# sudo-flow/zvec

Measured on AMD Instinct MI355X. Metric: QPS @ recall@10>=0.99, 10Mx768 fp32, batch=1024, higher is better.
Workload: dtype f32

## Files before the change

zvec_amd/csrc/api_entry_ctx_flat.inc.h:

```cpp

int zvec_hip_abi_version(void) { return ZVEC_HIP_ABI_VERSION; }

int zvec_hip_device_count(int *count) {
  if (!count) return ZVEC_HIP_ERR_INVALID_ARGUMENT;
  int n = 0;
  if (hipGetDeviceCount(&n) != hipSuccess) { *count = 0; return ZVEC_HIP_ERR_RUNTIME; }
  *count = n;
  return 0;
}

const char *zvec_hip_error_string(int code) {
  switch (code) {
    case ZVEC_HIP_OK: return "Success";
    case ZVEC_HIP_ERR_RUNTIME: return "Runtime error";
    case ZVEC_HIP_ERR_UNSUPPORTED: return "Unsupported";
    case ZVEC_HIP_ERR_OUT_OF_RANGE: return "Out of range";
    case ZVEC_HIP_ERR_NO_MEMORY: return "Not enough space";
    case ZVEC_HIP_ERR_NO_READY: return "No ready";
    case ZVEC_HIP_ERR_NO_EXIST: return "No exist";
    case ZVEC_HIP_ERR_MISMATCH: return "Mismatch";
    case ZVEC_HIP_ERR_INVALID_ARGUMENT: return "Invalid argument";
    case ZVEC_HIP_ERR_NO_INDEX_LOADED: return "No index loaded";
    case ZVEC_HIP_ERR_NO_TRAINED: return "No trained";
  }
  return "Unknown error";
}

int zvec_hip_set_option(const char *name, int value) {
  if (!name) return ZVEC_HIP_ERR_INVALID_ARGUMENT;
  if (strcmp(name, "wait") == 0) {
    if (value < 0 || value > 2) return ZVEC_HIP_ERR_INVALID_ARGUMENT;
    ropts().wait = value;
    return 0;
  }
  if (strcmp(name, "zerocopy") == 0) {
    if (value < 0 || value > 3) return ZVEC_HIP_ERR_INVALID_ARGUMENT;
    ropts().zerocopy = value;
    return 0;
  }
  if (strcmp(name, "assign256") == 0) { ropts().assign256 = value != 0; return 0; }
  if (strcmp(name, "scan256") == 0) {
    if (value < 0 || value > 2) return ZVEC_HIP_ERR_INVALID_ARGUMENT;
    ropts().scan256 = value;
    return 0;
  }
  if (strcmp(name, "sparse_group_rows") == 0) {
    if (value < 0 || value > 64) return ZVEC_HIP_ERR_INVALID_ARGUMENT;
    ropts().sparse_group_rows = value;
    return 0;
  }
  if (strcmp(name, "sparse_inverted_build") == 0) {
    if (value < 0 || value > 1) return ZVEC_HIP_ERR_INVALID_ARGUMENT;
    ropts().sparse_inverted_build = value;
    return 0;
  }
  return ZVEC_HIP_ERR_UNSUPPORTED;
}
int zvec_hip_get_option(const char *name, int *value) {
  if (!name || !value) return ZVEC_HIP_ERR_INVALID_ARGUMENT;
  if (strcmp(name, "wait") == 0) { *value = ropts().wait; return 0; }
  if (strcmp(name, "zerocopy") == 0) { *value = ropts().zerocopy; return 0; }
  if (strcmp(name, "assign256") == 0) { *value = ropts().assign256; return 0; }
  if (strcmp(name, "scan256") == 0) { *value = ropts().scan256; return 0; }
  if (strcmp(name, "sparse_group_rows") == 0) { *value = ropts().sparse_group_rows; return 0; }
  if (strcmp(name, "sparse_inverted_build") == 0) { *value = ropts().sparse_inverted_build; return 0; }
  return ZVEC_HIP_ERR_UNSUPPORTED;
}

int zvec_hip_host_alloc(uint64_t bytes, void **out) {
  if (!out || bytes == 0) return ZVEC_HIP_ERR_INVALID_ARGUMENT;
  void *p = nullptr;
  if (hipHostMalloc(&p, bytes, hipHostMallocPortable) != hipSuccess) { (void)hipGetLastError(); return ZVEC_HIP_ERR_NO_MEMORY; }
  *out = p;
  return 0;
}
int zvec_hip_host_free(void *p) {
  if (p) (void)hipHostFree(p);
  return 0;
}

int zvec_hip_ctx_create(int device, zvec_hip_ctx_t *out) {
  if (!out) return ZVEC_HIP_ERR_INVALID_ARGUMENT;
  return ctx_new(device, out);
}
int zvec_hip_ctx_destroy(zvec_hip_ctx_t ctx) { ctx_free(ctx); return 0; }
int zvec_hip_ctx_synchronize(zvec_hip_ctx_t ctx) {
  if (!ctx) return ZVEC_HIP_ERR_INVALID_ARGUMENT;
  ZCHK(hipSetDevice(ctx->device));
  ZCHK(hipStreamSynchronize(ctx->cur));
  return 0;
}
int zvec_hip_ctx_set_stream(zvec_hip_ctx_t ctx, void *stream) {
  if (!ctx) return ZVEC_HIP_ERR_INVALID_ARGUMENT;
  ctx->cur = stream ? reinterpret_cast<hipStream_t>(stream) : ctx->own;
  return 0;
}

int zvec_hip_gate_create(int device, zvec_hip_gate_t *out) {
  if (!out) return ZVEC_HIP_ERR_INVALID_ARGUMENT;
  ZCHK(hipSetDevice(device));
  zvec_hip_gate_s *g = new (std::nothrow) zvec_hip_gate_s();
  if (!g) return ZVEC_HIP_ERR_NO_MEMORY;
  g->device = device;
  if (hipEventCreateWithFlags(&g->ev, hipEventDisableTiming) != hipSuccess) { delete g; return ZVEC_HIP_ERR_RUNTIME; }
  *out = g;
  return 0;
}
int zvec_hip_gate_destroy(zvec_hip_gate_t g) {
  if (!g) return 0;
  (void)hipSetDevice(g->device);
  if (g->ev) (void)hipEventDestroy(g->ev);
  delete g;
  return 0;
}
int zvec_hip_ctx_set_gate(zvec_hip_ctx_t ctx, zvec_hip_gate_t gate) {
  if (!ctx || (gate && gate->device != ctx->device)) return ZVEC_HIP_ERR_INVALID_ARGUMENT;
  std::lock_guard<std::mutex> g(ctx->mu);
  ctx->gate = gate;
  return 0;
}

int zvec_hip_flat_create(uint32_t dim, int dtype, int metric, int device, zvec_hip_flat_t *out) {
  if (!out || dim == 0) return ZVEC_HIP_ERR_INVALID_ARGUMENT;
  if (dtype < ZVEC_HIP_DT_FP32 || dtype > ZVEC_HIP_DT_BINARY64) return ZVEC_HIP_ERR_UNSUPPORTED;
  if (metric < 0 || metric > ZVEC_HIP_METRIC_HAMMING) return ZVEC_HIP_ERR_UNSUPPORTED;
  if (dtype_is_binary(dtype) != (metric == ZVEC_HIP_METRIC_HAMMING)) return ZVEC_HIP_ERR_MISMATCH;
  if (dtype_is_binary(dtype) && (dim % (dtype == ZVEC_HIP_DT_BINARY64 ? 64u : 32u) != 0 || dim > (1u << 20))) return ZVEC_HIP_ERR_INVALID_ARGUMENT;
  if (metric == ZVEC_HIP_METRIC_COSINE && dim < (dtype == ZVEC_HIP_DT_FP16 ? 3u : 2u)) return ZVEC_HIP_ERR_INVALID_ARGUMENT;
  zvec_hip_ctx_s *c = nullptr;
  ZRET(ctx_new(device, &c));
  zvec_hip_flat_s *h = new (std::nothrow) zvec_hip_flat_s();
  if (!h) { ctx_free(c); return ZVEC_HIP_ERR_NO_MEMORY; }
  h->device = device; h->dtype = dtype; h->defctx = c;
  h->st.configure(dim, metric, dtype);
  *out = h;
  return 0;
}

int zvec_hip_flat_destroy(zvec_hip_flat_t h) {
  if (!h) return 0;
  (void)hipSetDevice(h->device);
  (void)hipDeviceSynchronize();
  delete h;
  return 0;
}

int zvec_hip_flat_reserve(zvec_hip_flat_t h, uint64_t capacity) {
  if (!h) return ZVEC_HIP_ERR_INVALID_ARGUMENT;
// ... 556 lines not shown
```

zvec_amd/csrc/api_flat_scan.inc.h:

```cpp

namespace {

struct KernelInfo {
  bool init = false;
  int cus = 0;
};
KernelInfo g_info[16];
std::mutex g_info_mu;

struct Knobs {
  int max_ng = 4;
  bool no_wide = false;
  bool force_wide = false;
  bool no_seed = false;
  bool no_gather = false;
  int ivf_tpc = 0;
  bool m16_small = true;
  int ivf_head_pct = 50;
  int ivf_occ_cap = 0;
  bool no_wide_dump = false;
  int ivf_direct_q = 8;
  int seed_rows256 = 16384;
  Knobs() {
#ifdef ZVEC_HIP_TUNING
    if (const char *e = getenv("ZVEC_HIP_MAX_NG")) max_ng = std::max(1, std::min(4, atoi(e)));
    no_wide = getenv("ZVEC_HIP_NO_WIDE") != nullptr;
    force_wide = getenv("ZVEC_HIP_FORCE_WIDE") != nullptr;
    no_seed = getenv("ZVEC_HIP_NO_SEED") != nullptr;
    no_gather = getenv("ZVEC_HIP_NO_GATHER") != nullptr;
    if (const char *e = getenv("ZVEC_HIP_IVF_TPC")) ivf_tpc = std::max(1, atoi(e));
    m16_small = getenv("ZVEC_HIP_NO_M16_SMALL") == nullptr;
    no_wide_dump = getenv("ZVEC_HIP_NO_WIDE_DUMP") != nullptr;
    if (const char *e = getenv("ZVEC_HIP_IVF_OCC_CAP")) ivf_occ_cap = std::max(0, atoi(e));
    if (const char *e = getenv("ZVEC_HIP_IVF_HEAD_PCT")) ivf_head_pct = std::max(0, std::min(75, atoi(e)));
    if (const char *e = getenv("ZVEC_HIP_IVF_DIRECT_Q")) ivf_direct_q = std::max(0, atoi(e));
    if (const char *e = getenv("ZVEC_HIP_SEED_ROWS256")) seed_rows256 = std::max(128, atoi(e) / 128 * 128);
#endif
  }
};
const Knobs &knobs() {
  static const Knobs k;
  return k;
}

template <auto Kernel>
int raise_dynamic_lds(size_t bytes) {
  static std::atomic<bool> done[16];
  int dev = 0;
  (void)hipGetDevice(&dev);
  std::atomic<bool> &d = done[dev & 15];
  if (!d.load(std::memory_order_acquire)) {
    ZCHK(hipFuncSetAttribute(reinterpret_cast<const void *>(Kernel), hipFuncAttributeMaxDynamicSharedMemorySize, (int)bytes));
    d.store(true, std::memory_order_release);
  }
  return 0;
}

template <int NG, bool M16, bool EXCL, bool F16>
int launch_scan_t(const ScanArgs &a, uint32_t max_items, int cus, hipStream_t stream) {
  size_t lds = scan_lds_bytes(NG, a.k, M16);
  ZRET((raise_dynamic_lds<&scan_kernel<NG, M16, EXCL, F16>>(LDS_LIMIT)));
  int occ = 0;
  ZCHK(hipOccupancyMaxActiveBlocksPerMultiprocessor(&occ, scan_kernel<NG, M16, EXCL, F16>, 256, lds));
  if (occ < 1) occ = 1;
  if (a.mode == 1 && knobs().ivf_occ_cap > 0) occ = std::min(occ, knobs().ivf_occ_cap);
  uint32_t grid = (uint32_t)std::min<uint64_t>((uint64_t)max_items, (uint64_t)cus * (uint64_t)occ);
  if (grid == 0) return 0;
  hipLaunchKernelGGL((scan_kernel<NG, M16, EXCL, F16>), dim3(grid), dim3(256), lds, stream, a);
  ZCHK(hipGetLastError());
  return 0;
}

template <int NG, bool M16>
int launch_scan(const ScanArgs &a, bool f16, uint32_t max_items, int cus, hipStream_t stream) {
  if (f16)
    return a.exclude ? launch_scan_t<NG, M16, true, true>(a, max_items, cus, stream)
                     : launch_scan_t<NG, M16, false, true>(a, max_items, cus, stream);
  return a.exclude ? launch_scan_t<NG, M16, true, false>(a, max_items, cus, stream)
                   : launch_scan_t<NG, M16, false, false>(a, max_items, cus, stream);
}

template <bool EXCL, bool F16, bool GATHER>
int launch_scan8_t(const ScanArgs &a, uint32_t max_items, int cus, hipStream_t stream, int *occ_out) {
  size_t lds = scan8_lds_bytes(a.k);
  ZRET((raise_dynamic_lds<&scan8_kernel<EXCL, F16, GATHER>>(LDS_LIMIT)));
  int occ = 0;
  ZCHK(hipOccupancyMaxActiveBlocksPerMultiprocessor(&occ, scan8_kernel<EXCL, F16, GATHER>, 512, lds));
  if (occ < 1) occ = 1;
  if (occ_out) { *occ_out = occ; return 0; }
  uint32_t grid = (uint32_t)std::min<uint64_t>((uint64_t)max_items, (uint64_t)cus * (uint64_t)occ);
  if (grid == 0) return 0;
  hipLaunchKernelGGL((scan8_kernel<EXCL, F16, GATHER>), dim3(grid), dim3(512), lds, stream, a);
  ZCHK(hipGetLastError());
  return 0;
}

int launch_scan8(const ScanArgs &a, bool f16, uint32_t max_items, int cus, hipStream_t stream, int *occ_out = nullptr) {
  if (a.gather_pos)
    return f16 ? launch_scan8_t<false, true, true>(a, max_items, cus, stream, occ_out)
               : launch_scan8_t<false, false, true>(a, max_items, cus, stream, occ_out);
  if (f16)
    return a.exclude ? launch_scan8_t<true, true, false>(a, max_items, cus, stream, occ_out)
                     : launch_scan8_t<false, true, false>(a, max_items, cus, stream, occ_out);
  return a.exclude ? launch_scan8_t<true, false, false>(a, max_items, cus, stream, occ_out)
                   : launch_scan8_t<false, false, false>(a, max_items, cus, stream, occ_out);
}

int launch_scan256_f16(const ScanArgs &a, uint32_t max_items, int cus, hipStream_t stream) {
  const size_t lds = scan256_lds_bytes(a.k);
  if (lds > LDS_LIMIT || a.nq < (uint32_t)S256_ROWS || a.nks < 2) return ZVEC_HIP_ERR_UNSUPPORTED;
  ZRET(raise_dynamic_lds<&scan256_f16_kernel>(LDS_LIMIT));
  const uint32_t grid = (uint32_t)std::min<uint64_t>((uint64_t)max_items, (uint64_t)cus);
  if (grid == 0) return 0;
  hipLaunchKernelGGL(scan256_f16_kernel, dim3(grid), dim3(512), lds, stream, a);
  ZCHK(hipGetLastError());
  return 0;
}

template <bool F16>
int launch_assign(const AssignArgs &a, int cus, hipStream_t s) {
  ZRET(raise_dynamic_lds<&assign_kernel<F16>>(ASSIGN_LDS));
  const uint32_t items = (a.nq + ASSIGN_ROWS - 1) / ASSIGN_ROWS;
  const uint32_t grid = std::min<uint32_t>(items, (uint32_t)cus * 2u);
  if (grid == 0) return 0;
  hipLaunchKernelGGL(assign_kernel<F16>, dim3(grid), dim3(256), ASSIGN_LDS, s, a);
  ZCHK(hipGetLastError());
  return 0;
}

template <bool L2>
int launch_assign256_f16_t(const AssignArgs &a, int cus, hipStream_t s) {
  ZRET(raise_dynamic_lds<&assign256_f16_kernel<L2>>(A256_LDS));
  const uint32_t items = (a.nq + A256_ROWS - 1) / A256_ROWS;
  const uint32_t grid = std::min<uint32_t>(items, (uint32_t)cus);
  if (grid == 0) return 0;
  hipLaunchKernelGGL(assign256_f16_kernel<L2>, dim3(grid), dim3(512), A256_LDS, s, a);
  ZCHK(hipGetLastError());
  return 0;
}
int launch_assign256_f16(const AssignArgs &a, int cus, hipStream_t s) {
  return a.metric == METRIC_L2 ? launch_assign256_f16_t<true>(a, cus, s) : launch_assign256_f16_t<false>(a, cus, s);
}

int launch_scan_ng(int ng, const ScanArgs &a, bool f16, uint32_t max_items, int cus, hipStream_t stream) {
  switch (ng) {
    case 0: return launch_scan<1, true>(a, f16, max_items, cus, stream);
    case 1: return launch_scan<1, false>(a, f16, max_items, cus, stream);
    case 2: return launch_scan<2, false>(a, f16, max_items, cus, stream);
    case 4: return launch_scan<4, false>(a, f16, max_items, cus, stream);
  }
  return ZVEC_HIP_ERR_INVALID_ARGUMENT;
}

int pick_ng(uint32_t rows_wanted, uint32_t k) {
  int ng = knobs().max_ng;
  while (ng > 1 && (uint32_t)(ng / 2) * QGROUP >= rows_wanted) ng /= 2;
  while (ng >= 1 && scan_lds_bytes(ng, k) > LDS_LIMIT - 1024) ng /= 2;
  return ng;
}

struct FlatSplit {
  uint32_t tpc = 1, nchunks = 1;
};
FlatSplit flat_split(uint64_t ntiles, uint32_t nqtiles, uint64_t resident) {
  FlatSplit f;
  const uint64_t slots_q = std::max<uint64_t>(1, (resident + nqtiles - 1) / nqtiles);
  uint64_t tpc = std::max<uint64_t>(1, (ntiles + slots_q - 1) / slots_q);
  tpc = std::max<uint64_t>(tpc, std::min<uint64_t>(ntiles, ntiles >= 4 * resident ? 4 : 1));
  f.tpc = (uint32_t)tpc;
  f.nchunks = (uint32_t)((ntiles + tpc - 1) / tpc);
  return f;
}

int device_cus(zvec_hip_ctx_s *ctx) {
  if (ctx->cus == 0) {
    hipDeviceProp_t prop;
    if (hipGetDeviceProperties(&prop, ctx->device) == hipSuccess) ctx->cus = prop.multiProcessorCount;
    if (ctx->cus <= 0) ctx->cus = 256;
  }
  return ctx->cus;
}

int prof_begin(zvec_hip_ctx_s *ctx, hipStream_t stream, double bytes, double flops, int is_ivf) {
  if (!ctx->profile || ctx->nprof >= PROFILE_MAX) return -1;
  int i = ctx->nprof;
  if ((int)ctx->ev0.size() <= i) {
    hipEvent_t a, b;
    if (hipEventCreate(&a) != hipSuccess || hipEventCreate(&b) != hipSuccess) return -1;
    ctx->ev0.push_back(a);
    ctx->ev1.push_back(b);
    ctx->host_bytes.push_back(0);
    ctx->host_flops.push_back(0);
    ctx->launch_is_ivf.push_back(0);
    ctx->prof_dscan.push_back(0);
  }
  ctx->host_bytes[i] = bytes;
  ctx->host_flops[i] = flops;
  ctx->launch_is_ivf[i] = is_ivf;
  (void)hipEventRecord(ctx->ev0[i], stream);
  return i;
}
void prof_end(zvec_hip_ctx_s *ctx, hipStream_t stream, int i) {
  if (i < 0) return;
  (void)hipEventRecord(ctx->ev1[i], stream);
  ctx->nprof = i + 1;
}

void gate_enter(zvec_hip_ctx_s *ctx, hipStream_t stream) {
  if (!ctx->gate) return;
  ctx->gate->mu.lock();
  if (ctx->gate->armed) (void)hipStreamWaitEvent(stream, ctx->gate->ev, 0);
}
void gate_leave(zvec_hip_ctx_s *ctx, hipStream_t stream) {
  if (!ctx->gate) return;
  (void)hipEventRecord(ctx->gate->ev, stream);
  ctx->gate->armed = true;
  ctx->gate->mu.unlock();
}

struct SearchOut {
  uint64_t *keys;
  float *scores;
  uint32_t *idx;
  uint32_t *counts;
};

int refine_l2(zvec_hip_ctx_s *ctx, const StoreView &st, uint32_t count, uint32_t topk, float threshold, uint64_t *keys,
              float *scores, uint32_t *idx, uint32_t *counts, hipStream_t stream);

inline uint32_t merge_threads(uint32_t count) { return count <= 256 ? 256u : 64u; }

inline size_t merge_lds_bytes(uint32_t k) { return (size_t)k * 12 + 16; }
constexpr size_t MERGE_LDS_MAX = 60 * 1024, SHARD_MERGE_LDS_MAX = 64 * 1024;
inline bool merge_fits(uint32_t k) { return merge_lds_bytes(k) <= MERGE_LDS_MAX; }
// ... 222 lines not shown
      if (can_gather) {
        const size_t padded = (size_t)(ktiles + 1) * TILE_N;
        ZRET(ctx->cmp_pos.ensure(padded * 4));
        ZCHK(hipMemsetAsync(ctx->cmp_pos.as<uint32_t>() + kept, 0, (padded - kept) * 4, stream));
        hipLaunchKernelGGL(keep_fill_kernel, dim3(nchunks_b), dim3(64), 0, stream, ex32, st.n, d_off, ctx->cmp_pos.as<uint32_t>());
        ZCHK(hipGetLastError());
        ZRET(flat_scan_gather(ctx, st, ctx->cmp_pos.as<uint32_t>(), kept, count, topk, threshold, out, stream, profile_it));
        if (user_facing) ZRET(refine_l2(ctx, st, count, topk, threshold, out.keys, out.scores, out.idx, out.counts, stream));
        return 0;
      }
      ZRET(ctx->cmp_pos.ensure((size_t)kept * 4));
      ZRET(ctx->cmp_base.ensure((size_t)ktiles * TILE_N * st.dpad * 4));
      ZRET(ctx->cmp_norm.ensure((size_t)ktiles * TILE_N * 4));
      ZRET(ctx->cmp_keys.ensure((size_t)ktiles * TILE_N * 8));
      if (st.extra) ZRET(ctx->cmp_extra.ensure((size_t)ktiles * TILE_N * 4));
      hipLaunchKernelGGL(keep_fill_kernel, dim3(nchunks_b), dim3(64), 0, stream, ex32, st.n, d_off, ctx->cmp_pos.as<uint32_t>());
      hipLaunchKernelGGL(compact_rows_kernel, dim3((kept + 3) / 4), dim3(256), 0, stream, st.base, st.bnorm, st.extra, st.keys,
                         ctx->cmp_pos.as<uint32_t>(), kept, st.dpad, ctx->cmp_base.as<float>(), ctx->cmp_norm.as<float>(),
                         st.extra ? ctx->cmp_extra.as<float>() : nullptr, ctx->cmp_keys.as<uint64_t>());
      ZCHK(hipGetLastError());
      StoreView tmp = st;
      tmp.base = ctx->cmp_base.as<float>(); tmp.bnorm = ctx->cmp_norm.as<float>();
      tmp.extra = st.extra ? ctx->cmp_extra.as<float>() : nullptr; tmp.keys = ctx->cmp_keys.as<uint64_t>();
      tmp.n = kept;
      return flat_scan_prepared(ctx, tmp, count, topk, threshold, nullptr, out_in, stream, role);
    }
  }
  {
    const uint64_t ntiles_d = (st.n + TILE_N - 1) / TILE_N;
    const double row_bytes_d = (double)ntiles_d * TILE_N * 4.0;
    const bool small_base = (double)st.n * st.dpad * 4.0 <= 64.0 * 1024 * 1024;
    const bool k_fits_merge = merge_fits(topk);
    const bool forced256 = ropts().scan256.load(std::memory_order_relaxed) == 2 && st.f16 && count >= (uint32_t)S256_ROWS &&
                           st.dpad / TILE_K >= 2 && scan256_lds_bytes(topk) <= LDS_LIMIT;
    const bool want_a = small_base && d_exclude == nullptr && topk > 8 && row_bytes_d * count <= 128.0 * 1024 * 1024 && !forced256;
    const bool want_b = pick_ng(count, topk) < 1;
    if (want_b && !k_fits_merge) return ZVEC_HIP_ERR_UNSUPPORTED;
    if ((want_a || want_b) && k_fits_merge) {
      const uint32_t sub = dense_sub_batch(count, ntiles_d * TILE_N);
      ZRET(ctx->part_s.ensure((size_t)ntiles_d * TILE_N * 4 * sub));
      for (uint32_t q0 = 0; q0 < count; q0 += sub) {
        const uint32_t cnt = std::min(sub, count - q0);
        float *dump = nullptr;
        uint32_t dump_stride = 0;
        ZRET(flat_dense_scores(ctx, st, q0, cnt, threshold, d_exclude, stream, &dump, &dump_stride));
        ZRET(launch_merge(merge_dense_rows(dump, dump_stride, topk, threshold, st.keys, out_from_row(out, q0, topk)), cnt, 64, stream));
      }
      if (user_facing) ZRET(refine_l2(ctx, st, count, topk, threshold, out.keys, out.scores, out.idx, out.counts, stream));
      return 0;
    }
  }
  const bool cache_resident = (double)st.n * st.dpad * 4.0 <= 64.0 * 1024 * 1024;
  const int opt256 = ropts().scan256.load(std::memory_order_relaxed);
  const bool can256 = opt256 != 0 && st.f16 && d_exclude == nullptr && count >= (uint32_t)S256_ROWS && st.dpad / TILE_K >= 2 &&
                      scan256_lds_bytes(topk) <= LDS_LIMIT && (uint64_t)count * st.dpad * 4ull < (1ull << 32);
  const bool wide = !knobs().no_wide && (!cache_resident || knobs().force_wide || (opt256 == 2 && can256)) && pick_ng(count, topk) == 4 &&
                    count > 2 * QGROUP && scan8_lds_bytes(topk) <= LDS_LIMIT - 1024;
  const bool wide256 = wide && can256;
  const uint64_t SEED_ROWS = wide256 ? (uint64_t)knobs().seed_rows256 : 4096;
  if (!knobs().no_seed && st.n >= 64 * 4096 && topk <= 64 && count >= 16) {
    SearchOut so;
    ZRET(seed_lists(ctx, count, topk, &so));
    StoreView view = st;
    view.n = SEED_ROWS;
    if (d_exclude == nullptr && (double)SEED_ROWS * 4.0 * count <= 256.0 * 1024 * 1024) {
      ZRET(ctx->part_s.ensure((size_t)SEED_ROWS * 4 * count));
      float *dump = nullptr;
      uint32_t dump_stride = 0;
      ZRET(flat_dense_scores(ctx, view, 0, count, threshold, nullptr, stream, &dump, &dump_stride));
      hipLaunchKernelGGL(seed_bound_kernel, dim3(count), dim3(256), 0, stream, dump, dump_stride, (uint32_t)SEED_ROWS, ctx->gtau.as<uint32_t>(),
                         ctx->qnorm.as<float>(), st.bnorm, st.metric, topk);
      ZCHK(hipGetLastError());
    } else {
      ZRET(flat_scan_prepared(ctx, view, count, topk, threshold, d_exclude, so, stream, ScanRole::internal));
      hipLaunchKernelGGL(seed_gtau_kernel, dim3((count + 255) / 256), dim3(256), 0, stream, ctx->gtau.as<uint32_t>(),
                         so.scores, so.idx, (const uint32_t *)nullptr, so.counts, ctx->qnorm.as<float>(), st.bnorm, st.metric, count, topk);
      ZCHK(hipGetLastError());
    }
  }
  int ng = pick_ng(count, topk);
  if (cache_resident && ng > 1) ng = 1;
  if (ng < 1) return ZVEC_HIP_ERR_UNSUPPORTED;
  const bool m16_small = knobs().m16_small && ng == 1 && count <= 16;
  const int cus = device_cus(ctx);
  int occ8 = 1;
  ScanArgs probe{};
  probe.k = topk; probe.exclude = reinterpret_cast<const uint32_t *>(d_exclude);
  if (wide && !wide256) ZRET(launch_scan8(probe, st.f16, 0, cus, stream, &occ8));
  const uint32_t rows = wide256 ? (uint32_t)S256_ROWS : wide ? W8_ROWS : ng * QGROUP;
  const uint32_t nqtiles = (count + rows - 1) / rows;
  const uint64_t ntiles = (st.n + TILE_N - 1) / TILE_N;
  uint64_t resident = wide256 ? (uint64_t)cus : wide ? (uint64_t)cus * occ8
                           : (uint64_t)cus * (ng >= 4 ? 2 : (ng == 2 ? 2 : 3));
  FlatSplit fs = flat_split(ntiles, nqtiles, resident);
  if (wide256 && (fs.tpc & 1)) {
    fs.tpc += 1;
    fs.nchunks = (uint32_t)((ntiles + fs.tpc - 1) / fs.tpc);
  }
  const uint64_t tpc = fs.tpc;
  uint32_t nchunks = fs.nchunks;
  uint64_t slots = (uint64_t)count * nchunks;
  ZRET(ctx->part_s.ensure(slots * topk * sizeof(float)));
  ZRET(ctx->part_i.ensure(slots * topk * sizeof(uint32_t)));

  ScanArgs a = scan_operands(ctx, st, d_exclude, threshold);
  a.k = topk; a.mode = 0; a.nq = count; a.n = st.n; a.ndense = st.n; a.tiles_per_chunk = (uint32_t)tpc; a.nchunks = nchunks; a.nqtiles = nqtiles;
  a.part_s = ctx->part_s.as<float>(); a.part_i = ctx->part_i.as<uint32_t>();
  int pi = -1;
  if (profile_it) {
    gate_enter(ctx, stream);
    pi = flat_prof_begin(ctx, st, st.n, count, topk, stream);
  }
  int lrc;
  if (wide256) lrc = launch_scan256_f16(a, ((nchunks + 7) / 8) * 8 * nqtiles, cus, stream);
  else if (wide) lrc = launch_scan8(a, st.f16, ((nchunks + 7) / 8) * 8 * nqtiles, cus, stream);
  else lrc = launch_scan_ng(m16_small ? 0 : ng, a, st.f16, nchunks * nqtiles, cus, stream);
  prof_end(ctx, stream, pi);
  if (profile_it) gate_leave(ctx, stream);
  ZRET(lrc);

  ZRET(launch_merge(merge_partials(a.part_s, a.part_i, nchunks, a.gtau, topk, threshold, st.keys, out), count, merge_threads(count), stream));
  if (user_facing) ZRET(refine_l2(ctx, st, count, topk, threshold, out.keys, out.scores, out.idx, out.counts, stream));
  return 0;
}

int refine_l2(zvec_hip_ctx_s *ctx, const StoreView &st, uint32_t count, uint32_t topk, float threshold, uint64_t *keys,
              float *scores, uint32_t *idx, uint32_t *counts, hipStream_t stream) {
  if (st.metric != ZVEC_HIP_METRIC_L2) return 0;
  if ((size_t)topk * 16 + 16 > 60 * 1024) return 0;
  const uint64_t pairs = (uint64_t)count * topk;
  if (st.f16)
    hipLaunchKernelGGL(rescore_l2_kernel<true>, dim3((unsigned)((pairs + 3) / 4)), dim3(256), 0, stream, st.base,
                       ctx->qpad.as<float>(), st.dpad, idx, counts, count, topk, scores, 1u);
  else
    hipLaunchKernelGGL(rescore_l2_kernel<false>, dim3((unsigned)((pairs + 3) / 4)), dim3(256), 0, stream, st.base,
                       ctx->qpad.as<float>(), st.dpad, idx, counts, count, topk, scores, 1u);
  hipLaunchKernelGGL(resort_kernel, dim3(count), dim3(64), (size_t)topk * 16 + 16, stream, keys, scores, idx, counts, topk,
                     threshold);
  ZCHK(hipGetLastError());
  return 0;
}

int prep_queries(zvec_hip_ctx_s *ctx, const StoreView &st, const void *d_queries, uint32_t count, float threshold,
                 hipStream_t stream) {
  ZRET(ctx->qpad.ensure((size_t)count * st.dpad * sizeof(float)));
  ZRET(ctx->qnorm.ensure((size_t)count * sizeof(float)));
  ZRET(ctx->gtau.ensure((size_t)count * sizeof(uint32_t)));
  if (st.bin) {
    const uint64_t words = (uint64_t)count * st.dpad;
    hipLaunchKernelGGL(hamming_prep_queries_kernel, dim3((unsigned)((words + 255) / 256)), dim3(256), 0, stream,
                       static_cast<const uint32_t *>(d_queries), count, st.bin_words(), st.bin_chunks(), ctx->qpad.as<uint32_t>(),
                       ctx->gtau.as<uint32_t>());
    ZCHK(hipGetLastError());
    return 0;
  }
  if (st.f16)
    hipLaunchKernelGGL(prep_queries_kernel<true>, dim3((count + 3) / 4), dim3(256), 0, stream, d_queries, count,
                       st.dim_in, st.dscan, st.dpad, ctx->qpad.as<float>(), ctx->qnorm.as<float>(),
                       ctx->gtau.as<uint32_t>(), threshold);
  else
    hipLaunchKernelGGL(prep_queries_kernel<false>, dim3((count + 3) / 4), dim3(256), 0, stream, d_queries, count,
                       st.dim_in, st.dscan, st.dpad, ctx->qpad.as<float>(), ctx->qnorm.as<float>(),
                       ctx->gtau.as<uint32_t>(), threshold);
  ZCHK(hipGetLastError());
  return 0;
}

int launch_pkeys_score(const StoreView &st, const void *queries, const uint32_t *d_pos, const uint32_t *d_off, uint32_t count,
                       uint32_t stride, float *part_s, uint32_t *part_i, hipStream_t stream) {
  const float *q = static_cast<const float *>(queries);
  if (st.bin)
    hipLaunchKernelGGL(hamming_pkeys_kernel, dim3((unsigned)(((uint64_t)count * stride + 255) / 256)), dim3(256), 0, stream,
                       reinterpret_cast<const uint32_t *>(st.base), static_cast<const uint32_t *>(queries), st.bin_chunks(), d_pos, d_off,
                       count, stride, part_s, part_i);
  else if (st.f16)
    hipLaunchKernelGGL(pkeys_score_kernel<true>, dim3(pkeys_score_blocks(count, stride)), dim3(256), 0, stream, st.base, q, st.dpad,
                       st.metric, d_pos, d_off, count, stride, part_s, part_i);
  else
    hipLaunchKernelGGL(pkeys_score_kernel<false>, dim3(pkeys_score_blocks(count, stride)), dim3(256), 0, stream, st.base, q, st.dpad,
                       st.metric, d_pos, d_off, count, stride, part_s, part_i);
  ZCHK(hipGetLastError());
  return 0;
}


int shadow_prep_queries(zvec_hip_ctx_s *ctx, const StoreView &twin, const void *d_queries, uint32_t count, hipStream_t stream) {
  ShadowScratch &sh = ctx->sh;
  ZRET(sh.q16.ensure((size_t)count * twin.dpad * sizeof(float)));
  ZRET(sh.qn16.ensure((size_t)count * sizeof(float)));
  ZRET(sh.qinfo.ensure((size_t)count * sizeof(f32x2)));
  hipLaunchKernelGGL(shadow_prep_queries_kernel, dim3((count + 3) / 4), dim3(256), 0, stream, reinterpret_cast<const float *>(d_queries),
                     count, twin.dim_in, twin.dscan, twin.dpad, sh.q16.as<float>(), sh.qn16.as<float>(), sh.qinfo.as<f32x2>());
  ZCHK(hipGetLastError());
  return 0;
}

int shadow_lists(zvec_hip_ctx_s *ctx, uint32_t count, uint32_t kp, SearchOut *pre) {
  ShadowScratch &sh = ctx->sh;
// ... 175 lines not shown
```

zvec_amd/csrc/api_types.inc.h:

```cpp

#define ZCHK(expr)                                                                               \
  do {                                                                                           \
    hipError_t _e = (expr);                                                                      \
    if (_e != hipSuccess) {                                                                      \
      fprintf(stderr, "[zvec_hip] %s failed: %s (%s:%d)\n", #expr, hipGetErrorString(_e),        \
              __FILE__, __LINE__);                                                               \
      return (_e == hipErrorOutOfMemory) ? ZVEC_HIP_ERR_NO_MEMORY : ZVEC_HIP_ERR_RUNTIME;        \
    }                                                                                            \
  } while (0)

#define ZRET(expr)            \
  do {                        \
    int _r = (expr);          \
    if (_r != 0) return _r;   \
  } while (0)

namespace {

constexpr size_t LDS_LIMIT = 160 * 1024;
constexpr int PROFILE_MAX = 8192;

template <typename T>
struct Scoped {
  T *p = nullptr;
  size_t cap = 0;
  Scoped() {}
  Scoped(Scoped &&o) noexcept : p(std::exchange(o.p, nullptr)), cap(std::exchange(o.cap, 0)) {}
  Scoped &operator=(Scoped &&o) noexcept { std::swap(p, o.p); std::swap(cap, o.cap); return *this; }
  ~Scoped() { release(); }
  int alloc_bytes(size_t bytes) {
    release();
    ZCHK(hipMalloc(reinterpret_cast<void **>(&p), bytes));
    cap = bytes;
    return 0;
  }
  int alloc(size_t count) { return alloc_bytes(count * sizeof(T)); }
  void release() { if (p) (void)hipFree(p); p = nullptr; cap = 0; }
  operator T *() const { return p; }
};

template <typename T>
int upload(Scoped<T> &d, const T *src, size_t n) {
  ZRET(d.alloc(std::max<size_t>(n, 1)));
  ZCHK(hipMemcpy(d, src, n * sizeof(T), hipMemcpyHostToDevice));
  return 0;
}

struct DevBuf : Scoped<void> {
  int ensure(size_t bytes) { return bytes <= cap ? 0 : alloc_bytes(bytes + bytes / 4 + 256); }
  template <typename T> T *as() const { return reinterpret_cast<T *>(p); }
};

struct DevView {
  void *p = nullptr;
  template <typename T> T *as() const { return reinterpret_cast<T *>(p); }
};

struct PinnedBuf {
  void *p = nullptr;
  void *dev = nullptr;
  size_t cap = 0;
  PinnedBuf() {}
  PinnedBuf(PinnedBuf &&o) noexcept { *this = std::move(o); }
  PinnedBuf &operator=(PinnedBuf &&o) noexcept { std::swap(p, o.p); std::swap(dev, o.dev); std::swap(cap, o.cap); return *this; }
  ~PinnedBuf() { release(); }
  int ensure(size_t bytes) {
    if (bytes <= cap) return 0;
    release();
    size_t want = bytes + bytes / 4 + 256;
    ZCHK(hipHostMalloc(&p, want, hipHostMallocMapped));
    if (hipHostGetDevicePointer(&dev, p, 0) != hipSuccess) { (void)hipGetLastError(); dev = nullptr; }
    cap = want;
    return 0;
  }
  void release() { if (p) (void)hipHostFree(p); p = nullptr; dev = nullptr; cap = 0; }
};

struct RuntimeOpts {
  std::atomic<int> wait{1};
  std::atomic<int> zerocopy{2};
  std::atomic<int> assign256{1};
  std::atomic<int> scan256{1};
  std::atomic<int> sparse_group_rows{32};
  std::atomic<int> sparse_inverted_build{1};
  RuntimeOpts() {
    if (const char *e = getenv("ZVEC_HIP_SCAN256")) scan256 = std::max(0, std::min(2, atoi(e)));
    if (const char *e = getenv("ZVEC_HIP_WAIT")) wait = std::max(0, std::min(2, atoi(e)));
    if (const char *e = getenv("ZVEC_HIP_ASSIGN256")) assign256 = atoi(e) != 0;
    if (const char *e = getenv("ZVEC_HIP_ZEROCOPY")) zerocopy = std::max(0, std::min(3, atoi(e)));
  }
};
inline RuntimeOpts &ropts() {
  static RuntimeOpts o;
  return o;
}

class FairSharedMutex {
 public:
  void lock() { gate_.lock(); rw_.lock(); gate_.unlock(); }
  void unlock() { rw_.unlock(); }
  void lock_shared() { gate_.lock(); rw_.lock_shared(); gate_.unlock(); }
  void unlock_shared() { rw_.unlock_shared(); }
 private:
  std::mutex gate_;
  std::shared_mutex rw_;
};

struct ShadowGovernor {
  std::atomic<uint32_t> bad{0}, pause{0}, clean{0};
  std::atomic<int> level{0}, floor_level{-8};
  uint32_t kp_auto(uint32_t topk) const {
    const int base = (int)std::max<uint32_t>(32, 3 * topk), lo = (int)std::max<uint32_t>(16, (topk * 3 / 2 + 7) / 8 * 8);
    return (uint32_t)std::min(64, std::max(lo, base + 8 * level.load(std::memory_order_relaxed)));
  }
  void report_width(uint32_t rerun, uint32_t count) {
    if (rerun == 0) {
      if (clean.fetch_add(1, std::memory_order_relaxed) + 1 >= 6) {
        clean.store(0, std::memory_order_relaxed);
        const int l = level.load(std::memory_order_relaxed);
        if (l > floor_level.load(std::memory_order_relaxed) && l > -4) level.store(l - 1, std::memory_order_relaxed);
      }
    } else {
      clean.store(0, std::memory_order_relaxed);
      if ((uint64_t)rerun * 32 > count) {
        const int l = level.load(std::memory_order_relaxed);
        floor_level.store(std::max(floor_level.load(std::memory_order_relaxed), l + 1), std::memory_order_relaxed);
        if (l < 4) level.store(l + 1, std::memory_order_relaxed);
      }
    }
  }
  bool allow() {
    uint32_t p = pause.load(std::memory_order_relaxed);
    while (p > 0 && !pause.compare_exchange_weak(p, p - 1, std::memory_order_relaxed)) {}
    return p == 0;
  }
  void report(uint32_t rerun, uint32_t count) {
    if ((uint64_t)rerun * 2 > count) {
      if (bad.fetch_add(1, std::memory_order_relaxed) + 1 >= 4) { bad.store(0, std::memory_order_relaxed); pause.store(64, std::memory_order_relaxed); }
    } else {
      bad.store(0, std::memory_order_relaxed);
    }
  }
  void reset() {
    bad.store(0, std::memory_order_relaxed); pause.store(0, std::memory_order_relaxed); clean.store(0, std::memory_order_relaxed);
    level.store(0, std::memory_order_relaxed); floor_level.store(-8, std::memory_order_relaxed);
  }
};

inline bool dtype_is_binary(int dtype) { return dtype == ZVEC_HIP_DT_BINARY32 || dtype == ZVEC_HIP_DT_BINARY64; }

struct StoreView {
  uint32_t dim_in = 0;
  uint32_t dscan = 0;
  uint32_t dpad = 0;
  uint32_t elem = 4;
  bool f16 = false;
  bool bin = false;
  int metric = 0;
  uint64_t n = 0;
  float *base = nullptr;
  float *bnorm = nullptr;
  float *extra = nullptr;
  uint64_t *keys = nullptr;

  void configure(uint32_t dim, int met, int dtype = ZVEC_HIP_DT_FP32) {
    dim_in = dim;
    metric = met;
    f16 = (dtype == ZVEC_HIP_DT_FP16);
// ... 344 lines not shown
```

zvec_amd/csrc/scan_kernels.hip.h:

```cpp
#pragma once
#include "zvk_common.hip.h"
#include "zvk_scan.hip.h"
#include "zvk_assign.hip.h"
#include "zvk_assign256.hip.h"
#include "zvk_scan256.hip.h"
#include "zvk_merge.hip.h"
#include "zvk_rows.hip.h"
#include "zvk_shadow.hip.h"
#include "zvk_filter.hip.h"
#include "zvk_plan.hip.h"
#include "zvk_build.hip.h"
#include "zvk_group.hip.h"
#include "zvk_hamming.hip.h"
#include "zvk_sparse.hip.h"
#include "zvk_sparse_inv.hip.h"
#include "zvk_sparse_invb.hip.h"
```

Baseline: 214,200.

## Add streaming flat-scan kernel for small-query L2 batches

Adds a new flat-scan kernel for L2 searches with at most four queries, no exclusions and ng==1. Each block grid-strides over base tiles with nontemporal loads and keeps query fragments in registers when the dimension fits. Distances are reduced with DPP lane sums, and each wave keeps its own top-k list in LDS before the waves merge. The path is on by default but only fires for tiny per-call query counts, so a batch of 1024 queries probably does not reach it.

```diff
diff --git a/zvec_amd/csrc/api_entry_ctx_flat.inc.h b/zvec_amd/csrc/api_entry_ctx_flat.inc.h
--- a/zvec_amd/csrc/api_entry_ctx_flat.inc.h
+++ b/zvec_amd/csrc/api_entry_ctx_flat.inc.h
@@ -54,6 +54,11 @@
     ropts().sparse_inverted_build = value;
     return 0;
   }
+  if (strcmp(name, "flat_stream") == 0) {
+    if (value < 0 || value > 1) return ZVEC_HIP_ERR_INVALID_ARGUMENT;
+    ropts().flat_stream = value;
+    return 0;
+  }
   return ZVEC_HIP_ERR_UNSUPPORTED;
 }
 int zvec_hip_get_option(const char *name, int *value) {
@@ -64,6 +69,7 @@
   if (strcmp(name, "scan256") == 0) { *value = ropts().scan256; return 0; }
   if (strcmp(name, "sparse_group_rows") == 0) { *value = ropts().sparse_group_rows; return 0; }
   if (strcmp(name, "sparse_inverted_build") == 0) { *value = ropts().sparse_inverted_build; return 0; }
+  if (strcmp(name, "flat_stream") == 0) { *value = ropts().flat_stream; return 0; }
   return ZVEC_HIP_ERR_UNSUPPORTED;
 }
 
diff --git a/zvec_amd/csrc/api_flat_scan.inc.h b/zvec_amd/csrc/api_flat_scan.inc.h
--- a/zvec_amd/csrc/api_flat_scan.inc.h
+++ b/zvec_amd/csrc/api_flat_scan.inc.h
@@ -21,6 +21,8 @@
   bool no_wide_dump = false;
   int ivf_direct_q = 8;
   int seed_rows256 = 16384;
+  int flat_stream_q = 4;
+  int flat_stream_wgs = 4;
   Knobs() {
 #ifdef ZVEC_HIP_TUNING
     if (const char *e = getenv("ZVEC_HIP_MAX_NG")) max_ng = std::max(1, std::min(4, atoi(e)));
@@ -35,6 +37,8 @@
     if (const char *e = getenv("ZVEC_HIP_IVF_HEAD_PCT")) ivf_head_pct = std::max(0, std::min(75, atoi(e)));
     if (const char *e = getenv("ZVEC_HIP_IVF_DIRECT_Q")) ivf_direct_q = std::max(0, atoi(e));
     if (const char *e = getenv("ZVEC_HIP_SEED_ROWS256")) seed_rows256 = std::max(128, atoi(e) / 128 * 128);
+    if (const char *e = getenv("ZVEC_HIP_FLAT_STREAM_Q")) flat_stream_q = std::max(0, std::min(FS_MAX_Q, atoi(e)));
+    if (const char *e = getenv("ZVEC_HIP_FLAT_STREAM_WGS")) flat_stream_wgs = std::max(1, atoi(e));
 #endif
   }
 };
@@ -150,6 +154,40 @@
     case 4: return launch_scan<4, false>(a, f16, max_items, cus, stream);
   }
   return ZVEC_HIP_ERR_INVALID_ARGUMENT;
+}
+
+template <int NQ, bool F16, bool QREG>
+int launch_flat_stream_t(const ScanArgs &a, hipStream_t stream, int *occ_out) {
+  const size_t lds = flat_stream_lds_bytes(NQ, a.k, a.dpad, QREG);
+  if (occ_out) {
+    int occ = 0;
+    ZCHK(hipOccupancyMaxActiveBlocksPerMultiprocessor(&occ, flat_stream_kernel<NQ, F16, QREG>, 256, lds));
+    *occ_out = std::max(occ, 1);
+    return 0;
+  }
+  hipLaunchKernelGGL((flat_stream_kernel<NQ, F16, QREG>), dim3(a.nchunks), dim3(256), lds, stream, a);
+  ZCHK(hipGetLastError());
+  return 0;
+}
+template <int NQ>
+int launch_flat_stream_q(const ScanArgs &a, bool f16, hipStream_t stream, int *occ_out) {
+  const bool qreg = NQ <= 4 && a.nks <= (uint32_t)FS_KB;
+  if constexpr (NQ <= 4) {
+    if (qreg) return f16 ? launch_flat_stream_t<NQ, true, true>(a, stream, occ_out) : launch_flat_stream_t<NQ, false, true>(a, stream, occ_out);
+  }
+  return f16 ? launch_flat_stream_t<NQ, true, false>(a, stream, occ_out) : launch_flat_stream_t<NQ, false, false>(a, stream, occ_out);
+}
+int launch_flat_stream(const ScanArgs &a, bool f16, hipStream_t stream, int *occ_out = nullptr) {
+  if (a.nq <= 1) return launch_flat_stream_q<1>(a, f16, stream, occ_out);
+  if (a.nq <= 2) return launch_flat_stream_q<2>(a, f16, stream, occ_out);
+  if (a.nq <= 4) return launch_flat_stream_q<4>(a, f16, stream, occ_out);
+  if (a.nq <= 8) return launch_flat_stream_q<8>(a, f16, stream, occ_out);
+  return ZVEC_HIP_ERR_INVALID_ARGUMENT;
+}
+bool flat_stream_route(const StoreView &st, uint32_t count, uint32_t topk, const uint64_t *d_exclude, int ng, bool user_facing) {
+  return ropts().flat_stream.load(std::memory_order_relaxed) != 0 && user_facing && st.metric == ZVEC_HIP_METRIC_L2 && !st.bin &&
+         d_exclude == nullptr && ng == 1 && topk <= FS_MAX_K && count <= (uint32_t)std::min(knobs().flat_stream_q, FS_MAX_Q) &&
+         flat_stream_lds_bytes(FS_MAX_Q, topk, st.dpad, false) <= 64 * 1024;
 }
 
 int pick_ng(uint32_t rows_wanted, uint32_t k) {
@@ -538,15 +576,22 @@
   if (cache_resident && ng > 1) ng = 1;
   if (ng < 1) return ZVEC_HIP_ERR_UNSUPPORTED;
   const bool m16_small = knobs().m16_small && ng == 1 && count <= 16;
+  const bool fstream = !wide && flat_stream_route(st, count, topk, d_exclude, ng, user_facing);
   const int cus = device_cus(ctx);
   int occ8 = 1;
   ScanArgs probe{};
   probe.k = topk; probe.exclude = reinterpret_cast<const uint32_t *>(d_exclude);
   if (wide && !wide256) ZRET(launch_scan8(probe, st.f16, 0, cus, stream, &occ8));
+  int occ_fs = 1;
+  if (fstream) {
+    probe.nq = count; probe.dpad = st.dpad; probe.nks = st.dpad / TILE_K;
+    ZRET(launch_flat_stream(probe, st.f16, stream, &occ_fs));
+    occ_fs = std::min(occ_fs, knobs().flat_stream_wgs);
+  }
   const uint32_t rows = wide256 ? (uint32_t)S256_ROWS : wide ? W8_ROWS : ng * QGROUP;
   const uint32_t nqtiles = (count + rows - 1) / rows;
   const uint64_t ntiles = (st.n + TILE_N - 1) / TILE_N;
-  uint64_t resident = wide256 ? (uint64_t)cus : wide ? (uint64_t)cus * occ8
+  uint64_t resident = wide256 ? (uint64_t)cus : wide ? (uint64_t)cus * occ8 : fstream ? (uint64_t)cus * occ_fs
                            : (uint64_t)cus * (ng >= 4 ? 2 : (ng == 2 ? 2 : 3));
   FlatSplit fs = flat_split(ntiles, nqtiles, resident);
   if (wide256 && (fs.tpc & 1)) {
@@ -570,6 +615,7 @@
   int lrc;
   if (wide256) lrc = launch_scan256_f16(a, ((nchunks + 7) / 8) * 8 * nqtiles, cus, stream);
   else if (wide) lrc = launch_scan8(a, st.f16, ((nchunks + 7) / 8) * 8 * nqtiles, cus, stream);
+  else if (fstream) lrc = launch_flat_stream(a, st.f16, stream);
   else lrc = launch_scan_ng(m16_small ? 0 : ng, a, st.f16, nchunks * nqtiles, cus, stream);
   prof_end(ctx, stream, pi);
   if (profile_it) gate_leave(ctx, stream);
diff --git a/zvec_amd/csrc/api_types.inc.h b/zvec_amd/csrc/api_types.inc.h
--- a/zvec_amd/csrc/api_types.inc.h
+++ b/zvec_amd/csrc/api_types.inc.h
@@ -83,7 +83,9 @@
   std::atomic<int> scan256{1};
   std::atomic<int> sparse_group_rows{32};
   std::atomic<int> sparse_inverted_build{1};
+  std::atomic<int> flat_stream{1};
   RuntimeOpts() {
+    if (const char *e = getenv("ZVEC_HIP_FLAT_STREAM")) flat_stream = atoi(e) != 0;
     if (const char *e = getenv("ZVEC_HIP_SCAN256")) scan256 = std::max(0, std::min(2, atoi(e)));
     if (const char *e = getenv("ZVEC_HIP_WAIT")) wait = std::max(0, std::min(2, atoi(e)));
     if (const char *e = getenv("ZVEC_HIP_ASSIGN256")) assign256 = atoi(e) != 0;
diff --git a/zvec_amd/csrc/scan_kernels.hip.h b/zvec_amd/csrc/scan_kernels.hip.h
--- a/zvec_amd/csrc/scan_kernels.hip.h
+++ b/zvec_amd/csrc/scan_kernels.hip.h
@@ -1,6 +1,7 @@
 #pragma once
 #include "zvk_common.hip.h"
 #include "zvk_scan.hip.h"
+#include "zvk_flat_stream.hip.h"
 #include "zvk_assign.hip.h"
 #include "zvk_assign256.hip.h"
 #include "zvk_scan256.hip.h"
diff --git a/zvec_amd/csrc/zvk_flat_stream.hip.h b/zvec_amd/csrc/zvk_flat_stream.hip.h
--- /dev/null
+++ b/zvec_amd/csrc/zvk_flat_stream.hip.h
@@ -0,0 +1,182 @@
+#pragma once
+#include "zvk_common.hip.h"
+
+namespace zvk {
+
+constexpr uint32_t FS_MAX_K = 64;
+constexpr int FS_MAX_Q = 8;
+constexpr int FS_KB = 4;
+constexpr int FS_PIECES = 4;
+
+__host__ __device__ inline size_t flat_stream_lds_bytes(int nq, uint32_t k, uint32_t dpad, bool qreg) {
+  return ((qreg ? 0 : (size_t)nq * dpad) + 4 * (size_t)nq * (2 * (size_t)k + 2)) * 4;
+}
+
+__device__ __forceinline__ float fs_row_sum(float v) {
+  v += __builtin_bit_cast(float, __builtin_amdgcn_update_dpp(0, __builtin_bit_cast(int, v), 0xB1, 0xf, 0xf, true));
+  v += __builtin_bit_cast(float, __builtin_amdgcn_update_dpp(0, __builtin_bit_cast(int, v), 0x4E, 0xf, 0xf, true));
+  v += __builtin_bit_cast(float, __builtin_amdgcn_update_dpp(0, __builtin_bit_cast(int, v), 0x141, 0xf, 0xf, true));
+  return v;
+}
+
+template <bool F16>
+__device__ __forceinline__ float fs_dot(const f32x4 b, const f32x4 q, float acc) {
+  if constexpr (F16) {
+    const f16x8 hb = __builtin_bit_cast(f16x8, b), hq = __builtin_bit_cast(f16x8, q);
+#pragma unroll
+    for (int e = 0; e < 8; ++e) acc = fmaf((float)hb[e], (float)hq[e], acc);
+  } else {
+    acc = fmaf(b.x, q.x, acc);
+    acc = fmaf(b.y, q.y, acc);
+    acc = fmaf(b.z, q.z, acc);
+    acc = fmaf(b.w, q.w, acc);
+  }
+  return acc;
+}
+
+template <int NQ, bool F16, bool QREG>
+__global__ void __launch_bounds__(256) flat_stream_kernel(const ScanArgs a) {
+  extern __shared__ f32x4 zvk_smem4[];
+  float *smem = reinterpret_cast<float *>(zvk_smem4);
+  const uint32_t dpad = a.dpad, nks = a.nks, k = a.k;
+  float *Qs = smem;
+  float *Ls = Qs + (QREG ? 0 : (size_t)NQ * dpad);
+  uint32_t *Li = reinterpret_cast<uint32_t *>(Ls + 4 * NQ * k);
+  uint32_t *cnt_s = Li + 4 * NQ * k;
+  float *tau_s = reinterpret_cast<float *>(cnt_s + 4 * NQ);
+
+  const int tid = threadIdx.x, lane = tid & 63, wave = tid >> 6;
+  const int p = lane & 7;
+  const int c = p ^ ((4 * (wave & 1) + (lane >> 4)) & 7);
+  const uint32_t chunk = blockIdx.x;
+  const uint32_t ntiles_total = (uint32_t)((a.n + TILE_N - 1) / TILE_N);
+
+  f32x4 qr[QREG ? NQ : 1][FS_KB];
+  float qn[NQ], tl[NQ], tg[NQ];
+  uint32_t cn[NQ];
+#pragma unroll
+  for (int q = 0; q < NQ; ++q) {
+    const bool live = (uint32_t)q < a.nq;
+    const uint32_t qi = live ? (uint32_t)q : 0u;
+    qn[q] = a.qnorm[qi];
+    tl[q] = live ? a.threshold : -__builtin_inff();
+    tg[q] = live ? fkey_inv(__hip_atomic_load(&a.gtau[qi], __ATOMIC_RELAXED, __HIP_MEMORY_SCOPE_AGENT)) : tl[q];
+    cn[q] = 0;
+    if constexpr (QREG) {
+#pragma unroll
+      for (int j = 0; j < FS_KB; ++j)
+        qr[q][j] = (uint32_t)j < nks ? *reinterpret_cast<const f32x4 *>(a.queries + (size_t)qi * dpad + (size_t)j * TILE_K + c * 4)
+                                     : f32x4{0.f, 0.f, 0.f, 0.f};
+    }
+  }
+  if constexpr (!QREG) {
+    for (uint32_t i = tid; i < (uint32_t)NQ * (dpad / 4); i += 256) {
+      const uint32_t q = i / (dpad / 4), w4 = i - q * (dpad / 4);
+      reinterpret_cast<f32x4 *>(Qs)[i] = reinterpret_cast<const f32x4 *>(a.queries + (size_t)(q < a.nq ? q : 0u) * dpad)[w4];
+    }
+    __syncthreads();
+  }
+
+  const int psel = p & 3;
+  const uint32_t row_in_tile = 8u * (uint32_t)(wave + 4 * psel) + (uint32_t)(lane >> 3);
+
+  for (uint32_t tile = chunk; tile < ntiles_total; tile += a.nchunks) {
+    const f32x4 *tb = reinterpret_cast<const f32x4 *>(a.base + (size_t)tile * TILE_N * dpad) + wave * 64 + lane;
+    const uint32_t pos = tile * TILE_N + row_in_tile;
+    const bool valid = p < 4 && (uint64_t)pos < a.n;
+    const float bn = valid ? a.bnorm[pos] : 0.f;
+
+    float acc[FS_PIECES][NQ];
+#pragma unroll
+    for (int g = 0; g < FS_PIECES; ++g)
+#pragma unroll
+      for (int q = 0; q < NQ; ++q) acc[g][q] = 0.f;
+
+    for (uint32_t kb = 0; kb < nks; kb += FS_KB) {
+      f32x4 v[FS_KB][FS_PIECES];
+#pragma unroll
+      for (int j = 0; j < FS_KB; ++j) {
+        const uint32_t ks = min(kb + (uint32_t)j, nks - 1);
+#pragma unroll
+        for (int g = 0; g < FS_PIECES; ++g) v[j][g] = __builtin_nontemporal_load(tb + (size_t)ks * (SLAB / 4) + g * 256);
+      }
+#pragma unroll
+      for (int j = 0; j < FS_KB; ++j) {
+        const uint32_t ks = min(kb + (uint32_t)j, nks - 1);
+#pragma unroll
+        for (int q = 0; q < NQ; ++q) {
+          f32x4 qv;
+          if constexpr (QREG) {
+            qv = qr[q][j];
+          } else {
+            qv = *reinterpret_cast<const f32x4 *>(Qs + (size_t)q * dpad + (size_t)ks * TILE_K + c * 4);
+            if (kb + j >= nks) qv = f32x4{0.f, 0.f, 0.f, 0.f};
+          }
+#pragma unroll
+          for (int g = 0; g < FS_PIECES; ++g) acc[g][q] = fs_dot<F16>(v[j][g], qv, acc[g][q]);
+        }
+      }
+    }
+
+#pragma unroll
+    for (int q = 0; q < NQ; ++q) {
+#pragma unroll
+      for (int g = 0; g < FS_PIECES; ++g) acc[g][q] = fs_row_sum(acc[g][q]);
+      const float dot = psel == 0 ? acc[0][q] : psel == 1 ? acc[1][q] : psel == 2 ? acc[2][q] : acc[3][q];
+      const float sc = fmaxf(fmaf(-2.f, dot, qn[q] + bn), 0.f);
+      float t = fminf(tl[q], tg[q]);
+      uint64_t m = __ballot(valid && sc <= t);
+      if (m == 0) continue;
+      float *L = Ls + (size_t)(wave * NQ + q) * k;
+      uint32_t *I = Li + (size_t)(wave * NQ + q) * k;
+      while (m != 0) {
+        const int l = __builtin_ctzll(m);
+        const float cs = bcast_f(sc, l);
+        const uint32_t ci = bcast_u(pos, l);
+        m &= m - 1;
+        if (sorted_insert<false>(L, nullptr, I, k, cn[q], cs, 0u, ci, lane, tl[q])) {
+          t = fminf(tl[q], tg[q]);
+          m &= __ballot(valid && sc <= t);
+        }
+      }
+    }
+  }
+
+  if (lane == 0) {
+#pragma unroll
+    for (int q = 0; q < NQ; ++q) {
+      cnt_s[wave * NQ + q] = cn[q];
+      tau_s[wave * NQ + q] = tl[q];
+    }
+  }
+  __syncthreads();
+#pragma unroll
+  for (int q = 0; q < NQ; ++q) {
+    if ((q & 3) != wave || (uint32_t)q >= a.nq) continue;
+    float *L = Ls + (size_t)q * k;
+    uint32_t *I = Li + (size_t)q * k;
+    uint32_t c0 = cnt_s[q];
+    float t0 = tau_s[q];
+    for (int w2 = 1; w2 < 4; ++w2) {
+      const uint32_t c2 = cnt_s[w2 * NQ + q];
+      const bool have = (uint32_t)lane < c2;
+      const float s = have ? Ls[(size_t)(w2 * NQ + q) * k + lane] : 0.f;
+      const uint32_t i = have ? Li[(size_t)(w2 * NQ + q) * k + lane] : 0u;
+      uint64_t m = __ballot(have && s <= t0);
+      while (m != 0) {
+        const int l = __builtin_ctzll(m);
+        const float cs = bcast_f(s, l);
+        const uint32_t ci = bcast_u(i, l);
+        m &= m - 1;
+        if (sorted_insert<false>(L, nullptr, I, k, c0, cs, 0u, ci, lane, t0)) m &= __ballot(have && s <= t0);
+      }
+    }
+    if ((uint32_t)lane < k) {
+      const size_t o = ((size_t)q * a.nchunks + chunk) * k + lane;
+      a.part_s[o] = (uint32_t)lane < c0 ? L[lane] : __builtin_inff();
+      a.part_i[o] = (uint32_t)lane < c0 ? I[lane] : IDX_NONE;
+    }
+  }
+}
+
+}
```

Result: slower. 212,000 (-1.0%).
